# vannem95/operational-space-control

Measured on AMD Instinct MI355X. Metric: OSC control steps/sec (batched envs), Go2 18-DoF, at 1/2/4/8 MI355X, higher is better.
Workload: dtype f64; 1 GPU; unitree_go2 standing mask=ones, 4096 envs per GPU (BASELINE configs[1]); robot=unitree_go2, envs_per_gpu=4096, global_envs=4096, parallelism=env-shard x1

## Files before the change

operational-space-control_amd/csrc/osc_ipm.hpp:

```cpp
#pragma once
#include "osc_internal.hpp"
#include "osc_ipm_ldl.hpp"
#include "osc_ipm_lds.hpp"
#include "osc_ipm_rows.hpp"
#include "osc_ipm_wheel.hpp"

namespace osc {

template <class D, bool SMALL, bool WARM, int RF_ = kRfNone, int CP = kCpNone>
__device__ __forceinline__ void ipm_block(
    const DevParams* __restrict__ P, int blk, int nenv, const double* __restrict__ gmask,
    const double* __restrict__ ws, double* __restrict__ gtau, double* __restrict__ gx,
    int32_t* __restrict__ gstatus, int32_t* __restrict__ giters, double* __restrict__ gwarm,
    int flags, double* __restrict__ sm, ParkArgs PA = ParkArgs{}) {
  static_assert(CP == kCpNone || (!WARM && RF_ == kRfFused && !D::WH),
                "compaction: cold solves with the fused refinement only");
  constexpr int NV = D::NV, NU = D::NU, NC = D::NC, NY = D::NY, NY1P = D::NY1P, MI = D::MI,
                NRL = D::NRL;
  const bool fixup = (flags & 1) != 0;
  const bool want_dual = (flags & 2) != 0;
  constexpr bool kFix = WARM || RF_ == kRfFused;
  constexpr int RF = RF_;
  constexpr bool REFINE = RF == kRfOnly;
  constexpr bool HRL = ipm_hrl<D, SMALL, RF>();
  using LY = IpmLayout<D, HRL>;
  const int lane = threadIdx.x;
  const int grp = lane / kRow, l = lane % kRow;
  const int cnt = CP == kCpResume ? *PA.count : nenv;
  if (CP == kCpResume && blk * kEnvPerWave >= cnt) return;
  const int env_raw = blk * kEnvPerWave + grp;
  const bool valid = env_raw < cnt;
  const int env = CP == kCpResume ? PA.list[valid ? env_raw : cnt - 1]
                                  : (valid ? env_raw : nenv - 1);
  bool write_out = valid;
  if constexpr (kFix) {
    const bool redo = valid && fixup && gstatus[env] != OSC_SOLVE_OK;
    if (fixup && __ballot(redo) == 0) return;
    write_out = valid && (!fixup || redo);
  }

  constexpr bool HRH = ipm_hrh<D, SMALL, RF>();
  constexpr int kEnvLds = LY::IL + refine_lds_extra<D, SMALL, RF>() + hrh_lds_extra<D, SMALL, RF>();
  double* B = sm + grp * kEnvLds;
  double* sHh = B + LY::IL + refine_lds_extra<D, SMALL, RF>();
  constexpr bool kXinHr = RF == kRfFused && HRL;
  double* sRX = kXinHr ? B + LY::I_HR : B + LY::IL + RefineLds<D>::X;
  double* sRH = kXinHr ? B + LY::IL : B + LY::IL + RefineLds<D>::HD;
  double* sRG = sRH + (RefineLds<D>::GD - RefineLds<D>::HD);
  constexpr bool kRefG = RF == kRfFused && (!SMALL || D::WH);
  constexpr bool WHR = D::WH && RF == kRfFused;
  using WL = WheelLds<D>;
  WheelRot W = wheel_rot<D>(B + LY::IL);
  const double* __restrict__ wsw =
      ws + (CP == kCpResume ? size_t{0} : static_cast<size_t>(blk) * kEnvPerWave * D::WS) +
      D::W_HR;
  const unsigned lane_off =
      static_cast<unsigned>(CP == kCpResume ? env : env - blk * kEnvPerWave) *
      static_cast<unsigned>(D::WS);
  double* sG = B + LY::I_G;
  double* sVy = B + LY::I_VY;
  double* sVy2 = B + LY::I_VY2;
  double* sVr = B + LY::I_VR;
  double* sDr = B + LY::I_DR;
  double* sMask = B + LY::I_MASK;
  double* sTau = B + LY::I_TAU;
  double* sXb = B + LY::I_XB;

  STAMP_DECL
  STAMP_BEGIN();
  static_assert(LY::STAGE % 2 == 0 && NC <= kRow, "staging layout");
  {
    Batch2<LY::STAGE / 2, kRow> bs;
    bs.load(ws + static_cast<size_t>(env) * D::WS, l);
    const double mk = gmask[static_cast<size_t>(env) * NC + (l < NC ? l : 0)];
    if constexpr (RF == kRfFused && !kRefG && !kXinHr) {
      static_assert(RefineLds<D>::SIZE % 2 == 0 && D::W_X % 2 == 0, "16-byte staging");
      Batch2<RefineLds<D>::SIZE / 2, kRow> bx;
      bx.load(ws + static_cast<size_t>(env) * D::WS + D::W_X, l);
      bx.store(sRX, l);
    }
    if constexpr (WHR) {
      const double* we = ws + static_cast<size_t>(env) * D::WS;
#pragma unroll 8
      for (int p = l; p < NY * NY; p += kRow) W.T[(p / NY) * WL::TST + p % NY] = we[D::W_T + p];
      for (int p = l; p < NY; p += kRow) W.Pin[p] = we[D::W_PIN + p];
      if (l < D::NW) {
        W.Q1[l] = we[D::W_AW + l * NY1P + NY];
        W.Nu[l] = 0.0;
      }
    }
    bs.store(B, l);
    if (l < NC) sMask[l] = mk;
  }
  const double* sHr = B + LY::I_HR;
  if constexpr (HRL && D::HRC) {
    const int ca = l, cb = l + kRow < NY ? l + kRow : NY - 1;
    const double* src = wsw + lane_off;
    if constexpr (kXinHr) {
      static_assert(D::HR_SIZE % 2 == 0 && D::HR_SIZE <= refine_lds_extra<D, SMALL, RF>() &&
                    D::W_HR % 2 == 0, "compact Hr staged in the refinement region");
      Batch2<D::HR_SIZE / 2, kRow> bh;
      bh.load(ws + static_cast<size_t>(env) * D::WS + D::W_HR, l);
      bh.store(B + LY::IL, l);
      wave_sync();
      src = B + LY::IL;
    }
#pragma unroll
    for (int i0 = 0; i0 < NY; i0 += 8) {
      double hv0[8], hv1[8];
#pragma unroll
      for (int i = 0; i < 8; ++i) {
        hv0[i] = i0 + i < NY ? src[hr_off<D>(i0 + i, ca)] : 0.0;
        hv1[i] = i0 + i < NY ? src[hr_off<D>(i0 + i, cb)] : 0.0;
      }
#pragma unroll
      for (int i = 0; i < 8; ++i) {
        if (i0 + i < NY) {
          const_cast<double*>(sHr)[(i0 + i) * NY + ca] = hv0[i];
          if (l + kRow < NY) const_cast<double*>(sHr)[(i0 + i) * NY + cb] = hv1[i];
        }
      }
    }
  }
  if constexpr (HRH) {
    static_assert(NY % 2 == 0 && D::WS % 2 == 0 && D::W_HR % 2 == 0, "16-byte Hr row loads");
#pragma unroll
    for (int i0 = 0; i0 < NY; i0 += 8) {
      double hv[8];
#pragma unroll
      for (int i = 0; i < 8; ++i)
        hv[i] = i0 + i < NY ? wsw[lane_off + static_cast<unsigned>(hr_off<D>(i0 + i, l))] : 0.0;
#pragma unroll
      for (int i = 0; i < 8; ++i)
        if (i0 + i < NY) sHh[(i0 + i) * kRow + l] = hv[i];
    }
  }
  wave_sync();

  bool act[NRL];
  double h[NRL];
#pragma unroll
  for (int t = 0; t < NRL; ++t) {
    const int r = l + kRow * t;
    act[t] = false;
    h[t] = 0.0;
    if (r < 2 * NU) {
      const int q = r >> 1;
      const double sg = (r & 1) ? -1.0 : 1.0;
      const double bnd = (r & 1) ? P->u_lb[q] : P->u_ub[q];
      act[t] = fabs(bnd) < P->inf_thresh;
      h[t] = sg * bnd;
    } else if (r < MI) {
      const int k = (r - 2 * NU) / 6, rt = (r - 2 * NU) % 6;
      const double m = sMask[k];
      if (m != 0.0) {
        if (rt < 4) {
          act[t] = true;
        } else if (rt == 4) {
          const double lb = P->z_lb[2] * m;
          act[t] = fabs(lb) < P->inf_thresh;
          h[t] = -lb;
        } else {
          const double ub = P->z_ub[2] * m;
          act[t] = fabs(ub) < P->inf_thresh;
          h[t] = ub;
        }
      }
    }
  }
  const double mu_f = P->mu;
  auto init_ls = [&](int t) -> bool {
    const int r = l + kRow * t;
    return act[t] && !(r >= 2 * NU && (r - 2 * NU) % 6 == 5);
  };
  STAMP_END(0);

  const int j0 = l, j1 = l + kRow;
  const bool v1 = j1 < NY;
  const int jj1 = v1 ? j1 : NY - 1;
  const int jk0 = (j0 >= NU) ? (j0 - NU) / 3 : -1, jc0 = (j0 >= NU) ? (j0 - NU) % 3 : 0;
  const int jk1 = (v1 && j1 >= NU) ? (j1 - NU) / 3 : -1, jc1 = (j1 >= NU) ? (j1 - NU) % 3 : 0;
  const RowLane L{l, j0, j1, jj1, v1, jk0, jc0, jk1, jc1, mu_f};

  constexpr int NW = D::NW;
  double rq0 = 0.0, rq1 = 0.0, rwmax = 0.0;
  if constexpr (WHR) rot_load_pins<D>(W, L);
  rq0 = W.pin0 ? W.q10 : 0.0;
  rq1 = W.pin1 ? W.q11 : 0.0;

  double c0[NY], c1[NY];
  double dinv0, dinv1;
  constexpr bool kHrReg = SMALL && !HRL && !D::WH;
  double hr0[kHrReg ? NY : 1], hr1[kHrReg ? NY : 1];
  if constexpr (kHrReg) {
#pragma unroll
    for (int i = 0; i < NY; ++i) {
      hr0[i] = wsw[lane_off + static_cast<unsigned>(hr_off<D>(i, j0))];
      hr1[i] = wsw[lane_off + static_cast<unsigned>(hr_off<D>(i, jj1))];
    }
  }
  auto load_hr = [&]() {
    if constexpr (HRL) {
#pragma unroll
      for (int i = 0; i < NY; ++i) {
        c0[i] = sHr[i * NY + j0];
        c1[i] = sHr[i * NY + jj1];
      }
    } else if constexpr (kHrReg) {
#pragma unroll
      for (int i = 0; i < NY; ++i) {
        c0[i] = hr0[i];
        c1[i] = hr1[i];
      }
    } else if constexpr (HRH) {
      unsigned off = lane_off;
      asm volatile("" : "+v"(off));
      const double* p1 = wsw + off + hr_off<D>(jj1, 0);
#pragma unroll
      for (int i = 0; i < NY; ++i) c1[i] = p1[i];
#pragma unroll
      for (int i = 0; i < NY; ++i) c0[i] = sHh[i * kRow + l];
    } else {
      unsigned off = lane_off;
      asm volatile("" : "+v"(off));
      const double* p = wsw + off;
#pragma unroll
      for (int i = 0; i < NY; ++i) {
        c0[i] = p[hr_off<D>(i, j0)];
        c1[i] = p[hr_off<D>(i, jj1)];
      }
    }
  };
  const double hdg0 =
      HRL ? sHr[j0 * NY + j0] : wsw[lane_off + static_cast<unsigned>(hr_off<D>(j0, j0))];
  const double hdg1 =
      HRL ? sHr[jj1 * NY + jj1] : wsw[lane_off + static_cast<unsigned>(hr_off<D>(jj1, jj1))];
  load_hr();
  const double g0 = sG[j0], g1 = sG[jj1];
  double y0 = 0.0, y1 = 0.0;
  double s[NRL], lam[NRL];
#pragma unroll
  for (int t = 0; t < NRL; ++t) {
    s[t] = 1.0;
    lam[t] = 0.0;
  }
  double nact = 0.0;
#pragma unroll
  for (int t = 0; t < NRL; ++t) nact += act[t] ? 1.0 : 0.0;
  const double m_act = row_sum(nact);
  bool done = !valid;
  int32_t st = OSC_SOLVE_MAX_ITER;
  int it_done = 0;
  bool stalled = false;

  double rp[NRL];
#pragma unroll
  for (int t = 0; t < NRL; ++t) rp[t] = 0.0;
  constexpr bool kRdCarry = !D::WH;
  double rdc0 = 0.0, rdc1 = 0.0;
  bool rd_fresh = true, rd_have = false;
  bool warm = false;
  if (WARM && !fixup) {
    const double* w0 = gwarm + static_cast<size_t>(env) * D::WW;
    const double same = (l >= NC || w0[D::WW_M + l] == sMask[l]) ? 1.0 : 0.0;
    warm = row_min(same) == 1.0 && w0[0] == 1.0 && m_act > 0.0;
  }
  bool any_warm = false, all_warm = false;
  if constexpr (WARM) {
    any_warm = __ballot(warm) != 0;
    all_warm = __ballot(!warm) == 0;
  }
  const int pslot = env_raw < cnt ? env_raw : cnt - 1;
  auto park_at = [&](int slot) {
    return PA.park + static_cast<size_t>(slot) * park_doubles<D>();
  };
  auto resume_state = [&]() -> int {
    if constexpr (CP == kCpResume) {
      const double* pk = park_at(pslot);
      y0 = pk[l];
      y1 = pk[kRow + l];
#pragma unroll
      for (int t = 0; t < NRL; ++t) {
        s[t] = pk[2 * kRow + l + kRow * t];
        lam[t] = pk[2 * kRow + NRL * kRow + l + kRow * t];
        rp[t] = pk[2 * kRow + 2 * NRL * kRow + l + kRow * t];
      }
      rdc0 = pk[2 * kRow + 3 * NRL * kRow + l];
      rdc1 = pk[3 * kRow + 3 * NRL * kRow + l];
      rd_have = true;
      sVy[j0] = y0;
      if (v1) sVy[j1] = y1;
      wave_sync();
    }
    return PA.park_it;
  };
  bool parked = false;
  bool refined = false;
  const double eps_run = (kFix && fixup) ? fmin(P->eps_mu, 1e-12) : P->eps_mu;
  const int max_iter = P->max_iter, restart_iter = P->restart_iter;
  const int warm_restart = WARM ? P->warm_restart : 0;
  if constexpr (REFINE) {
    static_assert(D::W_SOL - D::W_X == RefineLds<D>::SIZE && D::W_X % 2 == 0 &&
                  RefineLds<D>::SIZE % 2 == 0, "refinement LDS block = workspace [X | H_dv | f_dv]");
    {
      Batch2<RefineLds<D>::SIZE / 2, kRow> bx;
      bx.load(ws + static_cast<size_t>(env) * D::WS + D::W_X, l);
      bx.store(sRX, l);
    }
    const double* sol = ws + static_cast<size_t>(env) * D::WS + D::W_SOL;
    y0 = sol[j0];
    y1 = v1 ? sol[j1] : 0.0;
#pragma unroll
    for (int t = 0; t < NRL; ++t) {
      const double q = sol[even(NY) + l + kRow * t];
      lam[t] = q;
      s[t] = q > 0.0 ? 0.0 : 1.0;
    }
    st = static_cast<int32_t>(sol[even(NY) + NRL * kRow]);
    sVy[j0] = y0;
    if (v1) sVy[j1] = y1;
    wave_sync();
  } else
  for (int it = CP == kCpResume ? resume_state() : (all_warm ? 0 : -1);; ++it) {
    STAMP_BEGIN();
    const bool init = it < 0;
    double mu = 0.0;
    if (WARM && it == 0 && any_warm) {
      const double* wst = gwarm + static_cast<size_t>(env) * D::WW;
      if (warm) {
        y0 = wst[D::WW_Y + j0];
        y1 = v1 ? wst[D::WW_Y + j1] : 0.0;
        sVy[j0] = y0;
        if (v1) sVy[j1] = y1;
      }
      wave_sync();
      wave_sync();
      if (warm) {
        const double dlt = P->warm_delta;
#pragma unroll
        for (int t = 0; t < NRL; ++t) {
          const double gy = Gv<D>(L, act, sVy, t);
          const double wl = wst[D::WW_L + l + kRow * t];
          s[t] = act[t] ? fmax(h[t] - gy, dlt) : 1.0;
          lam[t] = act[t] ? fmax(wl, dlt) : 0.0;
        }
      }
      double c0s = 0.0;
#pragma unroll
      for (int t = 0; t < NRL; ++t) c0s += act[t] ? s[t] * lam[t] : 0.0;
      const double mu0 = P->warm_center * row_sum(c0s) / fmax(m_act, 1.0);
      if (warm) {
#pragma unroll
        for (int t = 0; t < NRL; ++t) {
          if (act[t]) {
            lam[t] = fmax(lam[t], mu0 * recip(s[t]));
            s[t] = fmax(s[t], mu0 * recip(lam[t]));
          }
        }
      }
      if constexpr (WHR) {
        double yh0, yh1;
        rot_in<D>(W, L, y0, y1, yh0, yh1);
        rq0 = W.pin0 ? yh0 + W.q10 : 0.0;
        rq1 = W.pin1 ? yh1 + W.q11 : 0.0;
        rwmax = row_max(fmax(fabs(rq0), fabs(rq1)));
      }
    }
    bool restart = false;
    if (it == restart_iter || (WARM && any_warm && it == warm_restart)) {
      double cr = 0.0, lmax = 0.0;
#pragma unroll
      for (int t = 0; t < NRL; ++t) {
        cr += act[t] ? s[t] * lam[t] : 0.0;
        lmax = fmax(lmax, lam[t]);
      }
      const bool far = row_sum(cr) / fmax(m_act, 1.0) > 1e-6 && row_max(lmax) <= kRecentreLamMax;
      const bool mine = far && !done && it == (warm ? warm_restart : restart_iter);
      restart = __ballot(mine) != 0;
      if (restart) wave_sync();
      if (mine) {
#pragma unroll
        for (int t = 0; t < NRL; ++t) {
          const double slack = h[t] - Gv<D>(L, act, sVy, t);
          s[t] = act[t] ? fmax(slack, 0.0) + 1.0 : 1.0;
          lam[t] = act[t] ? 1.0 : 0.0;
        }
      }
    }
    if (!init) {
      double cs = 0.0;
#pragma unroll
      for (int t = 0; t < NRL; ++t) {
        if constexpr (SMALL) {
          double sl = s[t] * lam[t];
          in_vgpr(sl);
          cs += sl;
        } else {
          cs += act[t] ? s[t] * lam[t] : 0.0;
        }
      }
      mu = row_sum(cs) / fmax(m_act, 1.0);
      const bool fresh = it == 0 || mu <= 1e-6 || restart;
      rd_fresh = fresh || !rd_have;
      if (__ballot(fresh) != 0) {
        wave_sync();
#pragma unroll
        for (int t = 0; t < NRL; ++t) {
          const double r = act[t] ? Gv<D>(L, act, sVy, t) + s[t] - h[t] : 0.0;
          rp[t] = fresh ? r : rp[t];
        }
      }
      if constexpr (SMALL) {
        const bool stop = !done && mu <= eps_run && (!D::WH || rwmax <= P->wheel_tol);
        done = done || stop;
        st = stop ? OSC_SOLVE_OK : st;
        it_done = stop ? it : it_done;
      } else if (!done && mu <= eps_run && (!D::WH || rwmax <= P->wheel_tol)) {
        done = true;
        st = OSC_SOLVE_OK;
        it_done = it;
      }
      if constexpr (CP == kCpPark) {
        if (it == PA.park_it && __ballot(!done) != 0) {
          int slot = 0;
          if (!done && l == 0) slot = atomicAdd(PA.count, 1);
          slot = __shfl(slot, grp * kRow, kWave);
          if (!done) {
            double* pk = park_at(slot);
            pk[l] = y0;
            pk[kRow + l] = y1;
#pragma unroll
            for (int t = 0; t < NRL; ++t) {
              pk[2 * kRow + l + kRow * t] = s[t];
              pk[2 * kRow + NRL * kRow + l + kRow * t] = lam[t];
              pk[2 * kRow + 2 * NRL * kRow + l + kRow * t] = rp[t];
            }
            pk[2 * kRow + 3 * NRL * kRow + l] = rdc0;
            pk[3 * kRow + 3 * NRL * kRow + l] = rdc1;
            if (l == 0) PA.list[slot] = env;
            parked = true;
            done = true;
          }
        }
      }
      if (__ballot(!done) == 0 || it >= max_iter) {
        if (!done) it_done = it;
        break;
      }
    }
    double inv_s[NRL];
#pragma unroll
    for (int t = 0; t < NRL; ++t) {
      const int r = l + kRow * t;
      if constexpr (SMALL) {
        inv_s[t] = act[t] ? recip(s[t]) : 0.0;
        sVr[r] = lam[t];
      } else {
        inv_s[t] = act[t] ? (init ? 1.0 : recip(s[t])) : 0.0;
        sVr[r] = init ? 0.0 : (act[t] ? lam[t] : 0.0);
      }
      sDr[r] = init ? (init_ls(t) ? 1.0 : 0.0) : lam[t] * inv_s[t];
    }
    wave_sync();

    STAMP_END(1);
    STAMP_BEGIN();
    double rd0 = rdc0, rd1 = rdc1;
    if (!kRdCarry || init || __ballot(rd_fresh && !done) != 0) {
      double rn0, rn1;
      GTw2<D, SMALL>(L, sVr, rn0, rn1);
      if constexpr (WHR) rot_in<D>(W, L, rn0, rn1, rn0, rn1);
      rn0 += g0;
      rn1 += g1;
      if constexpr (WHR) {
        if (!init) {
          double yh0, yh1;
          rot_in<D>(W, L, y0, y1, yh0, yh1);
          dot_rows<NY>(rn0, rn1, yh0, yh1, c0, c1);
        }
      } else {
        if (!init) dot_rows<NY>(rn0, rn1, y0, y1, c0, c1);
      }
      rd0 = (!kRdCarry || rd_fresh) ? rn0 : rd0;
      rd1 = (!kRdCarry || rd_fresh) ? rn1 : rd1;
    }
    rd_have = true;
    double dg0 = hdg0, dg1 = hdg1, du = 0.0;
    STAMP_END(8);
    STAMP_BEGIN();
    if constexpr (WHR) {
      assemble_rot<D>(W, L, sDr, c0, c1, dg0, dg1);
    } else {
      static_assert(D::NU <= kRow, "torque variables in the first column slot");
      const double2 dd = *reinterpret_cast<const double2*>(sDr + 2 * (j0 < NU ? j0 : 0));
      du = (j0 < NU) ? dd.x + dd.y : 0.0;
      dg0 += du;
    }
    STAMP_END(9);
    STAMP_BEGIN();
    if constexpr (!WHR) add_contact_blocks<D>(L, sDr, c0, c1, dg0, dg1);
    wave_sync();
    STAMP_END(2);
    STAMP_BEGIN();
    ldl_rows<NY, SMALL>(c0, c1, B + LY::I_DINV, l, dinv0, dinv1, 1e-13 * dg0, 1e-13 * dg1, du);
    wave_sync();
    STAMP_END(3);

    double ds[NRL], dl[NRL], dsdl[NRL];
#pragma unroll
    for (int t = 0; t < NRL; ++t) ds[t] = dl[t] = dsdl[t] = 0.0;
    double dy0 = 0.0, dy1 = 0.0, sig_mu = 0.0, step = 1.0, a_aff = 1.0;
    const int npass = init ? 1 : 2;
    for (int pass = 0; pass < npass; ++pass) {
      STAMP_BEGIN();
#pragma unroll
      for (int t = 0; t < NRL; ++t) {
        const double rc = fma(s[t], lam[t], dsdl[t]) - sig_mu;
        sVr[l + kRow * t] = init ? (init_ls(t) ? h[t] : 0.0) : (rc - lam[t] * rp[t]) * inv_s[t];
      }
      wave_sync();
      GTw2<D, SMALL>(L, sVr, dy0, dy1);
      if constexpr (WHR) {
        rot_in<D>(W, L, dy0, dy1, dy0, dy1);
        dy0 = W.pin0 ? -rq0 : dy0 - rd0;
        dy1 = W.pin1 ? -rq1 : dy1 - rd1;
      } else {
        dy0 -= rd0;
        dy1 -= rd1;
      }
      STAMP_END(4);
      STAMP_BEGIN();
      ldl_solve_rows<NY>(c0, c1, dinv0, dinv1, dy0, dy1, l);
      if constexpr (WHR) rot_out<D>(W, L, dy0, dy1, dy0, dy1);
      sVy2[j0] = dy0;
      if (v1) sVy2[j1] = dy1;
      wave_sync();
      STAMP_END(5);
      STAMP_BEGIN();
      wave_sync();
      double rmax = 1.0;
      double gdy_all[NRL];
      if constexpr (SMALL) Gv_all<D>(L, act, sVy2, gdy_all);
#pragma unroll
      for (int t = 0; t < NRL; ++t) {
        const double rc = fma(s[t], lam[t], dsdl[t]) - sig_mu;
        const double gdy = SMALL ? gdy_all[t] : Gv<D>(L, act, sVy2, t);
        ds[t] = act[t] ? -rp[t] - gdy : 0.0;
        dl[t] = -(rc + lam[t] * ds[t]) * inv_s[t];
        const double inv_l = (act[t] && !init) ? recip1(lam[t]) : 0.0;
        rmax = fmax(rmax, fmax(-ds[t] * inv_s[t], -dl[t] * inv_l));
      }
      step = recip(row_max(rmax));
      if (pass == 0 && !init) {
        double ca = 0.0;
#pragma unroll
        for (int t = 0; t < NRL; ++t)
          ca += act[t] ? (s[t] + step * ds[t]) * (lam[t] + step * dl[t]) : 0.0;
        a_aff = step;
        const double mu_aff = row_sum(ca) / fmax(m_act, 1.0);
        const double q = mu_aff / fmax(mu, 1e-300);
        sig_mu = q * q * mu;
#pragma unroll
        for (int t = 0; t < NRL; ++t) dsdl[t] = ds[t] * dl[t];
        if constexpr (WHR) {
          if (!done && mu <= 1e-8 && step < 0.1 && rwmax <= P->wheel_tol) {
            done = true;
            st = OSC_SOLVE_OK;
            it_done = it;
            stalled = true;
          }
        }
      }
      wave_sync();
      STAMP_END(6);
    }
    STAMP_BEGIN();
    if (init) {
      y0 = dy0;
      y1 = dy1;
      double zmax = -1e300, nzmax = -1e300;
#pragma unroll
      for (int t = 0; t < NRL; ++t) {
        const double zr = -ds[t] - h[t];
        if (act[t]) {
          zmax = fmax(zmax, zr);
          nzmax = fmax(nzmax, -zr);
        }
      }
      const double ap = row_max(zmax);
      const double ad = row_max(nzmax);
#pragma unroll
      for (int t = 0; t < NRL; ++t) {
        const double zr = -ds[t] - h[t];
        s[t] = act[t] ? ((ap >= 0.0) ? -zr + 1.0 + ap : -zr) : 1.0;
        lam[t] = act[t] ? ((ad >= 0.0) ? zr + 1.0 + ad : zr) : 0.0;
      }
      if (m_act == 0.0 && !done) {
        done = true;
        st = OSC_SOLVE_OK;
        it_done = 0;
      }
    } else {
      const double eta =
          fixup ? 0.99
                : fmin(1.0 - 1e-5, fmax(0.99, fmax(1.0 - mu, 1.0 - 0.1 * (1.0 - a_aff))));
      const double alpha = done ? 0.0 : fmin(1.0, eta * step);
      y0 = fma(alpha, dy0, y0);
      y1 = fma(alpha, dy1, y1);
#pragma unroll
      for (int t = 0; t < NRL; ++t) {
        s[t] = act[t] ? fma(alpha, ds[t], s[t]) : 1.0;
        lam[t] = act[t] ? fma(alpha, dl[t], lam[t]) : 0.0;
        rp[t] *= 1.0 - alpha;
      }
      if constexpr (kRdCarry) {
        rdc0 = (1.0 - alpha) * rd0;
        rdc1 = (1.0 - alpha) * rd1;
      }
    }
    sVy[j0] = y0;
    if (v1) sVy[j1] = y1;
    load_hr();
    wave_sync();
    if constexpr (WHR) {
      double yh0, yh1;
      rot_in<D>(W, L, y0, y1, yh0, yh1);
      rq0 = W.pin0 ? yh0 + W.q10 : 0.0;
      rq1 = W.pin1 ? yh1 + W.q11 : 0.0;
      rwmax = row_max(fmax(fabs(rq0), fabs(rq1)));
    }
    STAMP_END(7);
  }
#ifdef OSC_STAMPS
  if constexpr (RF != kRfFused) STAMP_STORE();
#endif
  if constexpr (RF == kRfNone) {
    if (write_out) {
      double* sol = const_cast<double*>(ws) + static_cast<size_t>(env) * D::WS + D::W_SOL;
      sol[j0] = y0;
      if (v1) sol[j1] = y1;
#pragma unroll
      for (int t = 0; t < NRL; ++t)
        sol[even(NY) + l + kRow * t] = (act[t] && lam[t] > s[t]) ? lam[t] : 0.0;
      if (l == 0) sol[even(NY) + NRL * kRow] = static_cast<double>(st);
    }
  }

  if constexpr (CP == kCpPark) write_out = write_out && !parked;
  const int refine_steps = P->refine_steps;
  if constexpr (RF != kRfNone) {
    const bool mine = valid && (st == OSC_SOLVE_OK || (WHR && st == OSC_SOLVE_MAX_ITER));
    if (P->refine_steps > 0 && __ballot(mine) != 0) {
      const double dpen = P->refine_penalty * row_max(fmax(fabs(hdg0), fabs(hdg1)));
      const double ytol = 1e-9 * (1.0 + row_max(fmax(fabs(y0), v1 ? fabs(y1) : 0.0)));
      constexpr bool kOldWh = WHR;
      double Dr[NRL], mur[NRL];
      const double stol =
          D::WH ? 1e-6 * (1.0 + row_max(fmax(fabs(y0), v1 ? fabs(y1) : 0.0))) : -1.0;
#pragma unroll
      for (int t = 0; t < NRL; ++t) {
        const bool a = act[t] && (lam[t] > s[t] || s[t] <= stol);
        Dr[t] = a ? dpen : 0.0;
        mur[t] = a ? lam[t] : 0.0;
      }
      const double wu = 2.0 * (P->w_torque + P->w_reg), wz = 2.0 * P->w_reg;
      double ya0 = y0, ya1 = y1;
      bool viol_env = false;
      const double* wenv = ws + static_cast<size_t>(env) * D::WS;
      const double* rX = kRefG ? wenv + D::W_X : sRX;
      const double* rH = kRefG ? wenv + D::W_HD : sRH;
      const double* rG = kRefG ? wenv + D::W_GD : sRG;
      constexpr int kUr = kRefG ? 2 : 32;
      double dlast = 0.0;
      bool settled = false;
      const double yscale = row_max(fmax(fabs(y0), v1 ? fabs(y1) : 0.0));
      double yk0 = 0.0, yk1 = 0.0, dk = 0.0, nuk = 0.0;
      bool conv = false;
      for (int round = 0; round < (WHR ? 5 : kRefineRounds); ++round) {
        STAMP_BEGIN();
#ifdef OSC_STAMPS
        st_acc[10] += 1ull << 40;
#endif
        if (round > 0) {
          if constexpr (kXinHr) {
#pragma unroll
            for (int i = 0; i < NY; ++i) {
              c0[i] = wsw[lane_off + static_cast<unsigned>(hr_off<D>(i, j0))];
              c1[i] = wsw[lane_off + static_cast<unsigned>(hr_off<D>(i, jj1))];
            }
          } else {
            load_hr();
          }
        }
#pragma unroll
        for (int t = 0; t < NRL; ++t) sDr[l + kRow * t] = Dr[t];
        ya0 = y0;
        ya1 = y1;
        sVy[j0] = y0;
        if (v1) sVy[j1] = y1;
        wave_sync();
        double dg0 = hdg0, dg1 = hdg1, du = 0.0;
        if constexpr (WHR) {
          wave_sync();
          assemble_rot<D>(W, L, sDr, c0, c1, dg0, dg1);
        } else {
          const double2 dd = *reinterpret_cast<const double2*>(sDr + 2 * (j0 < NU ? j0 : 0));
          du = (j0 < NU) ? dd.x + dd.y : 0.0;
          dg0 += du;
        }
        if constexpr (!WHR) add_contact_blocks<D>(L, sDr, c0, c1, dg0, dg1);
        if constexpr (kXinHr) {
          constexpr int NCH = D::NV * D::NY1P / 2;
          constexpr int NT = (NCH + kWave - 1) / kWave;
          static_assert(D::NV * D::NY1P <= even(NY * NY) && D::W_X % 2 == 0 &&
                        NT * kWave * 2 <= even(NY * NY), "X (whole DMA rows) in Hr's region");
          if (round == 0) {
            asm volatile("s_waitcnt lgkmcnt(0)" ::: "memory");
            static_for<0, kEnvPerWave>([&](auto G) {
              constexpr int g = decltype(G)::value;
              const int eg = CP == kCpResume ? __builtin_amdgcn_readlane(env, g * kRow)
                             : (blk * kEnvPerWave + g < nenv ? blk * kEnvPerWave + g : nenv - 1);
              const double2* src =
                  reinterpret_cast<const double2*>(ws + static_cast<size_t>(eg) * D::WS + D::W_X);
              static_for<0, NT>([&](auto T) {
                constexpr int t = decltype(T)::value;
                const int c = lane + kWave * t < NCH ? lane + kWave * t : NCH - 1;
#if defined(__HIP_DEVICE_COMPILE__)
                __builtin_amdgcn_global_load_lds(src + c, sm + g * kEnvLds + LY::I_HR + 2 * kWave * t,
                                                 16, 0, 0);
#else
                (void)src;
                (void)c;
#endif
              });
              {
                constexpr int NCH2 = (RefineLds<D>::SIZE - RefineLds<D>::HD) / 2;
                constexpr int NT2 = (NCH2 + kWave - 1) / kWave;
                static_assert(NT2 * kWave * 2 == refine_lds_extra<D, SMALL, RF>() &&
                              D::W_HD == D::W_X + RefineLds<D>::HD && D::W_HD % 2 == 0,
                              "[H_dv | f_dv] (whole DMA rows) in the refinement region");
                const double2* src2 =
                    reinterpret_cast<const double2*>(ws + static_cast<size_t>(eg) * D::WS + D::W_HD);
                static_for<0, NT2>([&](auto T) {
                  constexpr int t = decltype(T)::value;
                  const int c = lane + kWave * t < NCH2 ? lane + kWave * t : NCH2 - 1;
#if defined(__HIP_DEVICE_COMPILE__)
                  __builtin_amdgcn_global_load_lds(src2 + c, sm + g * kEnvLds + LY::IL + 2 * kWave * t,
                                                   16, 0, 0);
#else
                  (void)src2;
                  (void)c;
#endif
                });
              }
            });
          }
        }
        wave_sync();
        ldl_rows<NY, SMALL>(c0, c1, B + LY::I_DINV, l, dinv0, dinv1, 1e-13 * dg0, 1e-13 * dg1, du);
        if constexpr (kXinHr) {
          if (round == 0) asm volatile("s_waitcnt vmcnt(0)" ::: "memory");
        }
        wave_sync();
        STAMP_END(8);
        STAMP_BEGIN();
        conv = false;
        for (int k = 0; k < (kOldWh ? refine_steps : kRefineMaxSteps); ++k) {
          const double* yv = sVy;
          if constexpr (WHR) {
            double yh0, yh1;
            rot_in<D>(W, L, ya0, ya1, yh0, yh1);
            rq0 = W.pin0 ? yh0 + W.q10 : 0.0;
            rq1 = W.pin1 ? yh1 + W.q11 : 0.0;
            sVy2[j0] = yh0;
            if (v1) sVy2[j1] = yh1;
            wave_sync();
            yv = sVy2;
          }
#pragma unroll
          for (int t = 0; t < (NV + kRow - 1) / kRow; ++t) {
            const int rr = l + kRow * t;
            if (rr < NV) {
              const double* xr = rX + rr * NY1P;
              double a = xr[NY];
#pragma unroll kUr
              for (int i = 0; i < NY; ++i) a = fma(xr[i], yv[i], a);
              sXb[rr] = a;
            }
          }
          wave_sync();
          double gxr[(NV + kRow - 1) / kRow];
#pragma unroll
          for (int t = 0; t < (NV + kRow - 1) / kRow; ++t) {
            const int rr = l + kRow * t;
            gxr[t] = 0.0;
            if (rr < NV) {
              const double* hr = rH + rr * NV;
              double a = rG[rr];
#pragma unroll kUr
              for (int i = 0; i < NV; ++i) a = fma(hr[i], sXb[i], a);
              gxr[t] = a;
            }
          }
          wave_sync();
#pragma unroll
          for (int t = 0; t < (NV + kRow - 1) / kRow; ++t)
            if (l + kRow * t < NV) sDr[l + kRow * t] = gxr[t];
#pragma unroll
          for (int t = 0; t < NRL; ++t) sVr[l + kRow * t] = mur[t];
          wave_sync();
          if constexpr (D::WH && RF == kRfFused) {
            const double* Vw = wenv + D::W_WV;
            double vg = 0.0;
            if (l < NW) {
#pragma unroll
              for (int j = 0; j < NV; ++j) vg = fma(Vw[l * NV + j], sDr[j], vg);
            }
            double corr[(NV + kRow - 1) / kRow];
#pragma unroll
            for (int t = 0; t < (NV + kRow - 1) / kRow; ++t) corr[t] = 0.0;
            static_for<0, NW>([&](auto W) {
              constexpr int w = decltype(W)::value;
              const double bw = bcast_guarded<w>(vg);
#pragma unroll
              for (int t = 0; t < (NV + kRow - 1) / kRow; ++t) {
                const int rr = l + kRow * t;
                corr[t] = fma(Vw[w * NV + (rr < NV ? rr : 0)], bw, corr[t]);
              }
            });
            wave_sync();
#pragma unroll
            for (int t = 0; t < (NV + kRow - 1) / kRow; ++t)
              if (l + kRow * t < NV) sDr[l + kRow * t] -= corr[t];
            wave_sync();
          }
          double r0 = (j0 < NU ? wu : wz) * ya0, r1 = (jj1 < NU ? wu : wz) * ya1;
          double gm0, gm1;
          if constexpr (WHR) {
            GTw2<D, SMALL>(L, sVr, gm0, gm1);
            r0 += gm0;
            r1 += gm1;
            rot_in<D>(W, L, r0, r1, r0, r1);
          }
#pragma unroll kUr
          for (int i = 0; i < NV; ++i) {
            r0 = fma(rX[i * NY1P + j0], sDr[i], r0);
            r1 = fma(rX[i * NY1P + jj1], sDr[i], r1);
          }
          if constexpr (!WHR) {
            GTw2<D, SMALL>(L, sVr, gm0, gm1);
            r0 += gm0;
            r1 += gm1;
          }
          if constexpr (WHR) {
            const double p0v = W.Pin[j0], p1v = W.Pin[jj1];
            if (p0v >= 0.0) W.Nu[static_cast<int>(p0v)] = -r0;
            if (v1 && p1v >= 0.0) W.Nu[static_cast<int>(p1v)] = -r1;
          }
          wave_sync();
          double R3[NRL];
#pragma unroll
          for (int t = 0; t < NRL; ++t) {
            R3[t] = (Dr[t] != 0.0) ? Gv<D>(L, act, sVy, t) - h[t] : 0.0;
            sVr[l + kRow * t] = Dr[t] * R3[t];
          }
          wave_sync();
          double b0, b1;
          GTw2<D, SMALL>(L, sVr, b0, b1);
          if constexpr (WHR) rot_in<D>(W, L, b0, b1, b0, b1);
          double d0 = -r0 - b0, d1 = -r1 - b1;
          if constexpr (WHR) {
            d0 = W.pin0 ? -rq0 : d0;
            d1 = W.pin1 ? -rq1 : d1;
          }
          ldl_solve_rows<NY>(c0, c1, dinv0, dinv1, d0, d1, l);
          if constexpr (WHR) {
            rot_out<D>(W, L, d0, d1, d0, d1);
            dlast = row_max(fmax(fabs(d0), v1 ? fabs(d1) : 0.0));
          }
          const bool frz = !kOldWh && conv;
          if (frz) {
            d0 = 0.0;
            d1 = 0.0;
          }
          sVy2[j0] = d0;
          if (v1) sVy2[j1] = d1;
          wave_sync();
#pragma unroll
          for (int t = 0; t < NRL; ++t)
            mur[t] += frz ? 0.0 : Dr[t] * (Gv<D>(L, act, sVy2, t) + R3[t]);
          ya0 += d0;
          ya1 += d1;
          wave_sync();
          sVy[j0] = ya0;
          if (v1) sVy[j1] = ya1;
          wave_sync();
          if constexpr (!kOldWh) {
            const double dn = row_max(fmax(fabs(d0), v1 ? fabs(d1) : 0.0));
            if (!frz) dlast = dn;
            conv = conv || (k + 1 >= refine_steps && dn <= 1e-10 * (1.0 + yscale));
            if (k + 1 >= refine_steps && __ballot(mine && !conv) == 0) break;
          }
        }
        double nviol = 0.0, vl = 0.0, gv[NRL];
#pragma unroll
        for (int t = 0; t < NRL; ++t) {
          gv[t] = Gv<D>(L, act, sVy, t) - h[t];
          vl = fmax(vl, (act[t] && Dr[t] == 0.0 && gv[t] > ytol) ? gv[t] : 0.0);
        }
        const double vbest = WHR ? 0.0 : row_max(vl);
#pragma unroll
        for (int t = 0; t < NRL; ++t) {
          const bool v = act[t] && Dr[t] == 0.0 && gv[t] > ytol && (WHR || gv[t] == vbest);
          Dr[t] = v ? dpen : Dr[t];
          nviol += v ? 1.0 : 0.0;
        }
        {
          const bool drops = WHR || vbest == 0.0;
          double mmax = 0.0, mlo = 0.0;
#pragma unroll
          for (int t = 0; t < NRL; ++t) {
            mmax = fmax(mmax, Dr[t] != 0.0 ? fabs(mur[t]) : 0.0);
            mlo = fmin(mlo, Dr[t] != 0.0 ? mur[t] : 0.0);
          }
          const double mtol = 1e-9 * (1.0 + row_max(mmax));
          const double mworst = WHR ? 0.0 : row_min(mlo);
#pragma unroll
          for (int t = 0; t < NRL; ++t) {
            const bool leave = drops && Dr[t] != 0.0 && mur[t] < -mtol && (WHR || mur[t] == mworst);
            Dr[t] = leave ? 0.0 : Dr[t];
            mur[t] = leave ? 0.0 : mur[t];
            nviol += leave ? 1.0 : 0.0;
          }
        }
        viol_env = mine && row_max(nviol) > 0.0;
        const bool more =
            viol_env || (mine && (kOldWh ? dlast > 1e-10 * (1.0 + yscale) : !conv));
        if (mine && !more && !settled) {
          settled = true;
          yk0 = ya0;
          yk1 = ya1;
          if constexpr (WHR) {
            dk = dlast;
            nuk = l < NW ? W.Nu[l] : 0.0;
          }
        }
        STAMP_END(11);
        if (__ballot(more && !settled) == 0) break;
      }
      if (settled) {
        ya0 = yk0;
        ya1 = yk1;
        viol_env = false;
        if constexpr (WHR) dlast = dk;
      }
      const double mv = fmax(fabs(ya0 - y0), v1 ? fabs(ya1 - y1) : 0.0);
      const double myr = row_max(fmax(fabs(y0), v1 ? fabs(y1) : 0.0));
      const double ok =
          (isfinite(ya0) && isfinite(ya1) &&
           (kOldWh ? (mv <= 0.1 * (1.0 + myr) && dlast <= 1e-10 * (1.0 + myr))
                : (settled && mv <= P->refine_max_move * (1.0 + myr)))) ? 1.0 : 0.0;
      double wres = 0.0;
      if constexpr (WHR) {
        double yh0, yh1;
        rot_in<D>(W, L, ya0, ya1, yh0, yh1);
        wres = row_max(fmax(W.pin0 ? fabs(yh0 + W.q10) : 0.0, W.pin1 ? fabs(yh1 + W.q11) : 0.0));
      }
      const bool keep = !viol_env && row_min(ok) == 1.0 && wres <= ytol;
      if (mine && keep) {
        y0 = ya0;
        y1 = ya1;
        refined = true;
        st = OSC_SOLVE_OK;
      }
      if (mine && !keep && st == OSC_SOLVE_OK && !(WHR && rwmax <= ytol && !stalled))
        st = OSC_SOLVE_UNREFINED;
#ifdef OSC_REFINE_DIAG
      if (mine && !keep)
        st = OSC_SOLVE_UNREFINED + 16 * (viol_env ? 1 : 0) + 32 * (row_min(ok) == 1.0 ? 0 : 1) +
             64 * (wres <= ytol ? 0 : 1) + 128 * (row_min(dlast <= 1e-10 * (1.0 + myr) ? 1.0 : 0.0) == 1.0 ? 0 : 1) +
             256 * (row_min(mv <= 0.1 * (1.0 + myr) ? 1.0 : 0.0) == 1.0 ? 0 : 1);
#endif
      if constexpr (D::WH)
        put_wheel_duals<D>(ws, env, l, want_dual, write_out,
                           (mine && keep && l < NW) ? (settled ? nuk : W.Nu[l]) : 0.0);
      wave_sync();
      sVy[j0] = y0;
      if (v1) sVy[j1] = y1;
      wave_sync();
    }
  }

#ifdef OSC_STAMPS
  if constexpr (RF == kRfFused) STAMP_STORE();
#endif
  if constexpr (D::WH) {
    if (!refined) put_wheel_duals<D>(ws, env, l, want_dual, write_out, 0.0);
  }
  if (REFINE && !refined) {
    if (write_out && l == 0 && gstatus && st == OSC_SOLVE_UNREFINED) gstatus[env] = st;
    write_out = false;
  }
  if (l < NU) {
    const double tq = sVy[l];
    sTau[l] = tq;
    if (write_out) gtau[static_cast<size_t>(env) * NU + l] = tq;
  }
  if (gx != nullptr) {
    const double* yv = sVy;
    if constexpr (WHR) {
      double yh0, yh1;
      rot_in<D>(W, L, y0, y1, yh0, yh1);
      sVy2[j0] = yh0;
      if (v1) sVy2[j1] = yh1;
      wave_sync();
      yv = sVy2;
    }
#pragma unroll
    for (int t = 0; t < (NV + kRow - 1) / kRow; ++t) {
      const int rr = l + kRow * t;
      if (rr < NV) {
        const double* xr = ws + static_cast<size_t>(env) * D::WS + D::W_X + rr * NY1P;
        double xb = xr[NY];
#pragma unroll
        for (int i = 0; i < NY; ++i) xb = fma(xr[i], yv[i], xb);
        sXb[rr] = xb;
      }
    }
  }
  wave_sync();
  const double fin = (isfinite(y0) && (!v1 || isfinite(y1))) ? 1.0 : 0.0;
  if (row_min(fin) == 0.0) st = OSC_SOLVE_NUMERICAL;
  if (write_out) {
    if (gx != nullptr) {
#pragma unroll
      for (int t = 0; t < 3; ++t) {
        const int idx = l + kRow * t;
        if (idx < D::NX) {
          double v;
          if (idx < NV) v = sXb[idx];
          else if (idx < NV + NU) v = sTau[idx - NV];
          else v = sVy[NU + idx - NV - NU];
          gx[static_cast<size_t>(env) * D::NX + idx] = v;
        }
      }
    }
    if (l == 0 && !REFINE) {
      if (gstatus) gstatus[env] = st;
      if (giters) giters[env] = (kFix && fixup) ? P->max_iter + it_done : it_done;
    }
    if (WARM && !REFINE) {
      double* wo = gwarm + static_cast<size_t>(env) * D::WW;
      wo[D::WW_Y + j0] = y0;
      if (v1) wo[D::WW_Y + j1] = y1;
#pragma unroll
      for (int t = 0; t < NRL; ++t) wo[D::WW_L + l + kRow * t] = lam[t];
      if (l < NC) wo[D::WW_M + l] = sMask[l];
      if (l == 0) wo[0] = (st == OSC_SOLVE_NUMERICAL) ? 0.0 : 1.0;
    }
  }
}

}

#include "osc_ipm_launch.hpp"
```

Baseline: 31.16 million solves/s.

## Add lean fused iterative-refinement loop for the in-HR-X non-wheeled path

Adds a specialized refinement loop for the fused, X-in-HR configuration without the refined G path. It batches the constraint evaluations through Gv_all, reads y as double2 pairs, accumulates several rows per lane in registers, and drops some barriers. The goal is to cut LDS traffic and sync overhead in the refinement iterations of each IPM solve. It duplicates the loop logic, which adds code size and register pressure and could shift numerical results slightly.

```diff
diff --git a/operational-space-control_amd/csrc/osc_ipm.hpp b/operational-space-control_amd/csrc/osc_ipm.hpp
--- a/operational-space-control_amd/csrc/osc_ipm.hpp
+++ b/operational-space-control_amd/csrc/osc_ipm.hpp
@@ -49,6 +49,7 @@
   double* sRG = sRH + (RefineLds<D>::GD - RefineLds<D>::HD);
   constexpr bool kRefG = RF == kRfFused && (!SMALL || D::WH);
   constexpr bool WHR = D::WH && RF == kRfFused;
+  constexpr bool kLean = kXinHr && !kRefG;
   using WL = WheelLds<D>;
   WheelRot W = wheel_rot<D>(B + LY::IL);
   const double* __restrict__ wsw =
@@ -765,6 +766,96 @@
         STAMP_END(8);
         STAMP_BEGIN();
         conv = false;
+        if constexpr (kLean) {
+        for (int k = 0; k < kRefineMaxSteps; ++k) {
+          constexpr int NT = (NV + kRow - 1) / kRow;
+          double R3[NRL];
+          {
+            double g3[NRL];
+            Gv_all<D>(L, act, sVy, g3);
+#pragma unroll
+            for (int t = 0; t < NRL; ++t) {
+              R3[t] = (Dr[t] != 0.0) ? g3[t] - h[t] : 0.0;
+              sVr[l + kRow * t] = mur[t];
+              sDr[l + kRow * t] = Dr[t] * R3[t];
+            }
+          }
+          int rr[NT];
+          double acc[NT];
+#pragma unroll
+          for (int t = 0; t < NT; ++t) {
+            rr[t] = (l + kRow * t < NV) ? l + kRow * t : 0;
+            acc[t] = rX[rr[t] * NY1P + NY];
+          }
+          static_assert(NY % 2 == 0 && LY::I_VY % 2 == 0, "y read as 16-byte pairs");
+#pragma unroll
+          for (int i = 0; i < NY; i += 2) {
+            const double2 yy = *reinterpret_cast<const double2*>(sVy + i);
+#pragma unroll
+            for (int t = 0; t < NT; ++t) {
+              acc[t] = fma(rX[rr[t] * NY1P + i], yy.x, acc[t]);
+              acc[t] = fma(rX[rr[t] * NY1P + i + 1], yy.y, acc[t]);
+            }
+          }
+#pragma unroll
+          for (int t = 0; t < NT; ++t)
+            if (l + kRow * t < NV) sXb[l + kRow * t] = acc[t];
+          wave_sync();
+#pragma unroll
+          for (int t = 0; t < NT; ++t) acc[t] = rG[rr[t]];
+#pragma unroll
+          for (int i = 0; i < NV; ++i) {
+            const double di = sXb[i];
+#pragma unroll
+            for (int t = 0; t < NT; ++t) acc[t] = fma(rH[rr[t] * NV + i], di, acc[t]);
+          }
+          wave_sync();
+#pragma unroll
+          for (int t = 0; t < NT; ++t)
+            if (l + kRow * t < NV) sXb[l + kRow * t] = acc[t];
+          wave_sync();
+          double r0 = (j0 < NU ? wu : wz) * ya0, r1 = (jj1 < NU ? wu : wz) * ya1;
+#pragma unroll
+          for (int i = 0; i < NV; ++i) {
+            r0 = fma(rX[i * NY1P + j0], sXb[i], r0);
+            r1 = fma(rX[i * NY1P + jj1], sXb[i], r1);
+          }
+          double gm0, gm1, b0, b1;
+          GTw2<D, SMALL>(L, sVr, gm0, gm1);
+          GTw2<D, SMALL>(L, sDr, b0, b1);
+          r0 += gm0;
+          r1 += gm1;
+          double d0 = -r0 - b0, d1 = -r1 - b1;
+          ldl_solve_rows<NY>(c0, c1, dinv0, dinv1, d0, d1, l);
+          const bool frz = conv;
+          if (frz) {
+            d0 = 0.0;
+            d1 = 0.0;
+          }
+          sVy2[j0] = d0;
+          if (v1) sVy2[j1] = d1;
+          wave_sync();
+          {
+            double gd[NRL];
+            Gv_all<D>(L, act, sVy2, gd);
+#pragma unroll
+            for (int t = 0; t < NRL; ++t) {
+              double inc = Dr[t] * (gd[t] + R3[t]);
+              in_vgpr(inc);
+              mur[t] += frz ? 0.0 : inc;
+            }
+          }
+          ya0 += d0;
+          ya1 += d1;
+          sVy[j0] = ya0;
+          if (v1) sVy[j1] = ya1;
+          wave_sync();
+          const double dn = row_max(fmax(fabs(d0), v1 ? fabs(d1) : 0.0));
+          if (!frz) dlast = dn;
+          conv = conv || (k + 1 >= refine_steps && dn <= 1e-10 * (1.0 + yscale));
+          if (k + 1 >= refine_steps && __ballot(mine && !conv) == 0) break;
+        }
+        } else
         for (int k = 0; k < (kOldWh ? refine_steps : kRefineMaxSteps); ++k) {
           const double* yv = sVy;
           if constexpr (WHR) {
@@ -903,9 +994,10 @@
           }
         }
         double nviol = 0.0, vl = 0.0, gv[NRL];
+        if constexpr (kLean) Gv_all<D>(L, act, sVy, gv);
 #pragma unroll
         for (int t = 0; t < NRL; ++t) {
-          gv[t] = Gv<D>(L, act, sVy, t) - h[t];
+          gv[t] = (kLean ? gv[t] : Gv<D>(L, act, sVy, t)) - h[t];
           vl = fmax(vl, (act[t] && Dr[t] == 0.0 && gv[t] > ytol) ? gv[t] : 0.0);
         }
         const double vbest = WHR ? 0.0 : row_max(vl);
```

Result: faster. 32.00 million solves/s, median of 6 (+2.7%).
